# facebookresearch/SlowFast

Hardware: NVIDIA H100
Metric: clips/sec (fwd+bwd) SlowFast-8x8-R50 (higher is better)
Workload: dtype bf16x3-split operands, f32 accumulate/storage

## Files before the change

### slowfast_b200/csrc/conv_igemm.cu

```cuda
#include <algorithm>
#include <cstdint>
#include <cstdio>

#include "../../include/slowfast_b200.h"
#include "ptx.cuh"
#include "runtime.h"

namespace sfb {

constexpr int BLOCK_M = 128;
constexpr int MAX_STAGES = 8;
constexpr int CONV_THREADS = 384;
constexpr int PRODUCER_REGS = 40;
constexpr int CONSUMER_REGS = 232;
constexpr int BAR_ORDER = 1;
constexpr int BAR_EPI = 3;
constexpr int BN_MAX = 128;
constexpr int BLOCK_K = 64;
constexpr int KSTEPS = BLOCK_K / 16;
constexpr long long kNoRow = INT64_MIN;
constexpr uint32_t EPI_SCRATCH = BLOCK_M * 8 + 4 * 8 * 32 * 4;
static_assert(4 * BN_MAX * 2 * 4 <= 4 * 8 * 32 * 4, "BatchNorm partials fit the staging blocks");

struct ConvParams {
  CUtensorMap tmA[2];
  CUtensorMap tmB[2];
  int M, oq, op, oz, nb;
  int sw, sh, sd;
  int lw, lh, ld;
  int kw, kh, kd;
  int dw, dh, dd;
  int CK, cpt, n_chunks, cps, k_blocks;
  int Ntot, BN, n_tiles, m_tiles;
  int ksplit;
  int stages;
  int a_tiled;
  uint32_t stage_bytes, chunk_bytes, b_bytes, a_total_bytes, a_plane_bytes;
  uint32_t a_layout, a_sbo, a_lbo;
  uint32_t a_kstep[KSTEPS];
  uint32_t off_epi, off_bars;
  float* out;
  long long os_n, os_z, os_p, os_q;
  int accumulate;
  float* stats;
};

__device__ __forceinline__ int k_block_begin(const ConvParams& p, int kpart) {
  return kpart * p.k_blocks / p.ksplit;
}

int conv_direct_try(const sfb_conv_desc* d, cudaStream_t stream, int* rc_out);

template <int BN, int MODE>
__device__ __forceinline__ void store_fragment(const float (&d)[2][BN / 2], float* stage, const long long* roff,
                                               float* out, int ncols) {
  const int warp = (threadIdx.x >> 5) & 3, lane = threadIdx.x & 31;
  const int g = lane >> 2, cq = 2 * (lane & 3);
  const int rr = lane >> 3, c4 = 4 * (lane & 7);
#pragma unroll
  for (int rb = 0; rb < 2; ++rb) {
#pragma unroll
    for (int h = 0; h < 2; ++h) {
#pragma unroll
      for (int cg = 0; cg < (BN + 31) / 32; ++cg) {
#pragma unroll
        for (int jj = 0; jj < 4; ++jj) {
          const int jn = 4 * cg + jj;
          if (jn < BN / 8)
            *reinterpret_cast<float2*>(stage + g * 32 + ((8 * jj + cq) ^ (8 * (g & 3)))) =
                make_float2(d[rb][4 * jn + 2 * h], d[rb][4 * jn + 2 * h + 1]);
        }
        __syncwarp();
        float4 v[2];
#pragma unroll
        for (int k = 0; k < 2; ++k) v[k] = *reinterpret_cast<const float4*>(stage + (rr + 4 * k) * 32 + (c4 ^ (8 * rr)));
        __syncwarp();
        const int col = 32 * cg + c4;
        if (col >= ncols) continue;
        float4* dst[2];
        bool ok[2];
#pragma unroll
        for (int k = 0; k < 2; ++k) {
          const long long o = roff[64 * rb + 16 * warp + 8 * h + rr + 4 * k];
          ok[k] = o != kNoRow;
          dst[k] = reinterpret_cast<float4*>(out + (ok[k] ? o + col : 0));
        }
        if (MODE == 1) {
          float4 o[2];
#pragma unroll
          for (int k = 0; k < 2; ++k)
            if (ok[k]) o[k] = *dst[k];
#pragma unroll
          for (int k = 0; k < 2; ++k)
            if (ok[k]) *dst[k] = make_float4(v[k].x + o[k].x, v[k].y + o[k].y, v[k].z + o[k].z, v[k].w + o[k].w);
        } else {
#pragma unroll
          for (int k = 0; k < 2; ++k) {
            if (!ok[k]) continue;
            if (MODE == 2)
              asm volatile("red.global.add.v4.f32 [%0], {%1, %2, %3, %4};" ::"l"(dst[k]), "f"(v[k].x), "f"(v[k].y),
                           "f"(v[k].z), "f"(v[k].w) : "memory");
            else
              *dst[k] = v[k];
          }
        }
      }
    }
  }
}

template <int NSPLIT, int BN>
__global__ void __launch_bounds__(CONV_THREADS, 1) conv_igemm_kernel(const __grid_constant__ ConvParams p) {
  static_assert(BN % 16 == 0 && BN <= BN_MAX, "tile width: a multiple of 16 up to BN_MAX");
  extern __shared__ uint8_t smem_raw[];
  uint8_t* smem = reinterpret_cast<uint8_t*>((reinterpret_cast<uintptr_t>(smem_raw) + 1023) & ~uintptr_t(1023));

  uint64_t* full = reinterpret_cast<uint64_t*>(smem + p.off_bars);
  uint64_t* empty = full + MAX_STAGES;

  if (threadIdx.x == 0) {
    for (int s = 0; s < p.stages; ++s) {
      mbar_init(&full[s], 1);
      mbar_init(&empty[s], 128);
    }
    fence_mbar_init();
    fence_proxy_async_smem();
  }
  __syncthreads();

  const int total_units = p.m_tiles * p.n_tiles * p.ksplit;

  if (threadIdx.x < 128) {
    setmaxnreg_dec<PRODUCER_REGS>();
    if (threadIdx.x >= 32) return;
    if (threadIdx.x == 0) {
      tma_prefetch_desc(&p.tmA[0]);
      tma_prefetch_desc(&p.tmB[0]);
      if (NSPLIT == 3) {
        tma_prefetch_desc(&p.tmA[1]);
        tma_prefetch_desc(&p.tmB[1]);
      }
    }
    int stage = 0;
    uint32_t phase = 0;
    for (int unit = blockIdx.x; unit < total_units; unit += gridDim.x) {
      const int tile = unit / p.ksplit, kpart = unit - tile * p.ksplit;
      const int mt = tile / p.n_tiles, nt = tile - mt * p.n_tiles;
      const int kb0 = k_block_begin(p, kpart), kb1 = k_block_begin(p, kpart + 1);
      int t = mt * BLOCK_M;
      const int q0 = t % p.oq;
      t /= p.oq;
      const int p0 = t % p.op;
      t /= p.op;
      const int z0 = t % p.oz;
      const int n0 = t / p.oz;
      const int cw = p.lw + q0 * p.sw, ch = p.lh + p0 * p.sh, cd = p.ld + z0 * p.sd;
      for (int kb = kb0; kb < kb1; ++kb) {
        mbar_wait(&empty[stage], phase ^ 1);
        if (elect_one()) {
          const int chunk0 = kb * p.cps;
          const uint32_t bytes = (uint32_t(p.cps) * p.chunk_bytes + p.b_bytes) * (NSPLIT == 3 ? 2u : 1u);
          mbar_expect_tx(&full[stage], bytes);
          uint8_t* st = smem + size_t(stage) * p.stage_bytes;
          for (int j = 0; j < p.cps; ++j) {
            const int idx = chunk0 + j;
            int nn = p.nb, c0 = 0;
            uint16_t ow = 0, oh = 0, od = 0;
            if (idx < p.n_chunks) {
              const int tap = idx / p.cpt;
              c0 = (idx - tap * p.cpt) * p.CK;
              const int tw = tap % p.kw;
              const int t2 = tap / p.kw;
              const int th = t2 % p.kh;
              const int td = t2 / p.kh;
              ow = uint16_t(tw * p.dw);
              oh = uint16_t(th * p.dh);
              od = uint16_t(td * p.dd);
              nn = n0;
            }
            if (p.a_tiled) {
              const int row0 = idx < p.n_chunks ? mt * BLOCK_M : p.m_tiles * BLOCK_M;
              tma_load_2d(st + j * p.chunk_bytes, &p.tmA[0], &full[stage], c0, row0);
              if (NSPLIT == 3) tma_load_2d(st + p.a_plane_bytes + j * p.chunk_bytes, &p.tmA[1], &full[stage], c0, row0);
              continue;
            }
            tma_load_im2col_5d(st + j * p.chunk_bytes, &p.tmA[0], &full[stage], c0, cw, ch, cd, nn, ow, oh, od);
            if (NSPLIT == 3)
              tma_load_im2col_5d(st + p.a_plane_bytes + j * p.chunk_bytes, &p.tmA[1], &full[stage], c0, cw, ch, cd,
                                 nn, ow, oh, od);
          }
          tma_load_2d(st + p.a_total_bytes, &p.tmB[0], &full[stage], kb * 64, nt * BN);
          if (NSPLIT == 3)
            tma_load_2d(st + p.a_total_bytes + p.b_bytes, &p.tmB[1], &full[stage], kb * 64, nt * BN);
        }
        __syncwarp();
        if (++stage == p.stages) {
          stage = 0;
          phase ^= 1;
        }
      }
    }
    return;
  }

  setmaxnreg_inc<CONSUMER_REGS>();
  const int c = (threadIdx.x >> 7) - 1;
  const int t = threadIdx.x & 127, warp = t >> 5, lane = t & 31;
  const uint32_t a_rb = (8u * p.a_sbo) >> 4;
  float d[2][BN / 2];
  int stage = 0;
  uint32_t phase = 0;
  for (int j = 0, unit = blockIdx.x; unit < total_units; ++j, unit += gridDim.x) {
    const int tile = unit / p.ksplit, kpart = unit - tile * p.ksplit;
    const int kb0 = k_block_begin(p, kpart), kb1 = k_block_begin(p, kpart + 1);
    if ((j & 1) != c) {
      for (int kb = kb0; kb < kb1; ++kb) {
        if (++stage == p.stages) {
          stage = 0;
          phase ^= 1;
        }
      }
      continue;
    }
    if (j > 0) named_bar_sync(BAR_ORDER + c, 256);
#pragma unroll
    for (int i = 0; i < BN / 2; ++i) d[0][i] = d[1][i] = 0.f;
    int held = -1;
    for (int kb = kb0; kb < kb1; ++kb) {
      mbar_wait(&full[stage], phase);
      wgmma_fence();
      const uint32_t a_base = smem_u32(smem + size_t(stage) * p.stage_bytes);
      const uint32_t b_base = a_base + p.a_total_bytes;
      const uint64_t a_hi0 = make_smem_desc(a_base, p.a_lbo, p.a_sbo, p.a_layout);
      const uint64_t b_hi0 = make_smem_desc(b_base, 16, 1024, 2);
#pragma unroll
      for (int ks = 0; ks < KSTEPS; ++ks) {
        const uint64_t a_hi = a_hi0 + p.a_kstep[ks];
        const uint64_t b_hi = b_hi0 + uint64_t(ks * 2);
        if (NSPLIT == 3) {
          const uint64_t a_lo = a_hi + (p.a_plane_bytes >> 4);
          const uint64_t b_lo = b_hi + (p.b_bytes >> 4);
          wgmma_m64n<BN>(d[0], a_lo, b_hi);
          wgmma_m64n<BN>(d[1], a_lo + a_rb, b_hi);
          wgmma_m64n<BN>(d[0], a_hi, b_lo);
          wgmma_m64n<BN>(d[1], a_hi + a_rb, b_lo);
        }
        wgmma_m64n<BN>(d[0], a_hi, b_hi);
        wgmma_m64n<BN>(d[1], a_hi + a_rb, b_hi);
      }
      wgmma_commit();
      wgmma_wait<1>();
      if (held >= 0) mbar_arrive(&empty[held]);
      held = stage;
      if (++stage == p.stages) {
        stage = 0;
        phase ^= 1;
      }
    }
    if (unit + int(gridDim.x) < total_units) named_bar_arrive(BAR_ORDER + (c ^ 1), 256);

    const int mt = tile / p.n_tiles, nt = tile - mt * p.n_tiles;
    const int ncol0 = nt * BN;
    uint8_t* epi = smem + p.off_epi + size_t(c) * EPI_SCRATCH;
    long long* roff_s = reinterpret_cast<long long*>(epi);
    {
      int r = mt * BLOCK_M + t;
      long long off = kNoRow;
      if (r < p.M) {
        const int oq_ = r % p.oq;
        r /= p.oq;
        const int op_ = r % p.op;
        r /= p.op;
        const int oz_ = r % p.oz;
        const int on_ = r / p.oz;
        off = on_ * p.os_n + oz_ * p.os_z + op_ * p.os_p + oq_ * p.os_q;
      }
      roff_s[t] = off;
    }
    named_bar_sync(BAR_EPI + c, 128);
    const int cq = 2 * (lane & 3);
    const int ncols = min(BN, ((p.Ntot + 3) & ~3) - ncol0);
    float* stage_w = reinterpret_cast<float*>(epi + BLOCK_M * 8) + warp * 256;
    wgmma_wait<0>();
    mbar_arrive(&empty[held]);
    if (p.accumulate == 2) store_fragment<BN, 2>(d, stage_w, roff_s, p.out + ncol0, ncols);
    else if (p.accumulate == 1) store_fragment<BN, 1>(d, stage_w, roff_s, p.out + ncol0, ncols);
    else store_fragment<BN, 0>(d, stage_w, roff_s, p.out + ncol0, ncols);
    if (p.stats != nullptr) {
      float* red = reinterpret_cast<float*>(epi + BLOCK_M * 8);
      named_bar_sync(BAR_EPI + c, 128);
#pragma unroll
      for (int jn = 0; jn < BN / 8; ++jn) {
        float s[2], q[2];
#pragma unroll
        for (int e = 0; e < 2; ++e) {
          const float a0 = d[0][4 * jn + e], a1 = d[0][4 * jn + 2 + e], a2 = d[1][4 * jn + e], a3 = d[1][4 * jn + 2 + e];
          s[e] = (a0 + a1) + (a2 + a3);
          q[e] = fmaf(a0, a0, fmaf(a1, a1, fmaf(a2, a2, a3 * a3)));
#pragma unroll
          for (int o = 4; o <= 16; o <<= 1) {
            s[e] += __shfl_xor_sync(0xffffffffu, s[e], o);
            q[e] += __shfl_xor_sync(0xffffffffu, q[e], o);
          }
        }
        if (lane < 4)
          *reinterpret_cast<float4*>(red + (size_t(warp) * BN + 8 * jn + cq) * 2) = make_float4(s[0], q[0], s[1], q[1]);
      }
      named_bar_sync(BAR_EPI + c, 128);
      const int col = ncol0 + t;
      if (t < BN && col < p.Ntot) {
        float s = 0.f, s2 = 0.f;
#pragma unroll
        for (int w = 0; w < 4; ++w) {
          s += red[(size_t(w) * BN + t) * 2 + 0];
          s2 += red[(size_t(w) * BN + t) * 2 + 1];
        }
        p.stats[size_t(col) * p.m_tiles + mt] = s;
        p.stats[(size_t(p.Ntot) + col) * p.m_tiles + mt] = s2;
      }
      named_bar_sync(BAR_EPI + c, 128);
    }
  }
}

static int pick_ck(int c) {
  if (c % 64 == 0) return 64;
  if (c % 32 == 0) return 32;
  if (c % 16 == 0) return 16;
  return 8;
}

struct ConvGrid {
  int64_t M;
  int CK, cps, n_chunks, k_blocks, BN, m_tiles, n_tiles;
};
static ConvGrid conv_grid(const sfb_conv_desc* d) {
  ConvGrid g;
  g.M = int64_t(d->n) * d->out_t * d->out_h * d->out_w;
  g.CK = pick_ck(d->c);
  g.cps = BLOCK_K / g.CK;
  g.n_chunks = d->kt * d->kh * d->kw * (d->c / g.CK);
  g.k_blocks = (g.n_chunks + g.cps - 1) / g.cps;
  g.BN = std::min((d->cout + 15) / 16 * 16, BN_MAX);
  g.m_tiles = int((g.M + BLOCK_M - 1) / BLOCK_M);
  g.n_tiles = (d->cout + g.BN - 1) / g.BN;
  return g;
}

static bool rows_regular(const sfb_conv_desc* d) {
  return d->os_h == int64_t(d->out_w) * d->os_w && d->os_t == int64_t(d->out_h) * d->os_h &&
         d->os_n == int64_t(d->out_t) * d->os_t;
}

static int conv_ksplit(const sfb_conv_desc* d, const ConvGrid& g, int P, bool with_stats) {
  const int tiles = g.m_tiles * g.n_tiles;
  if (P <= 0 || d->c <= 8 || 2 * tiles < P) return 1;
  if ((d->accumulate == 0 || with_stats) && !rows_regular(d)) return 1;
  if (with_stats && (d->accumulate != 0 || d->cout % 8 != 0 || d->os_w % 4 != 0)) return 1;
  auto cost = [&](int s) { return double((int64_t(tiles) * s + P - 1) / P) / s * (1.0 + 0.02 * (s - 1)); };
  int best = 1;
  for (int s = 2; s <= 8 && 4 * s <= g.k_blocks; ++s)
    if (cost(s) < cost(best)) best = s;
  return cost(best) < 0.9 * cost(1) ? best : 1;
}

}

using namespace sfb;

extern "C" int64_t sfb_conv_m_tiles(const sfb_conv_desc* d) {
  const ConvGrid g = conv_grid(d);
  int sms = 0;
  if (device_limits(&sms, nullptr) == 0 && conv_ksplit(d, g, sms, true) > 1)
    return sfb_bn_split_stats_tiles(g.M, g.M, 1, d->cout);
  return g.m_tiles;
}

extern "C" int32_t sfb_conv_ksplit(const sfb_conv_desc* d) {
  int sms = 0;
  if (device_limits(&sms, nullptr)) return 1;
  return conv_ksplit(d, conv_grid(d), sms, d->stats != nullptr);
}

extern "C" int sfb_conv_igemm(const sfb_conv_desc* d, void* stream_) {
  cudaStream_t stream = reinterpret_cast<cudaStream_t>(stream_);
  int num_sms = 0, smem_optin = 0;
  if (device_limits(&num_sms, &smem_optin)) return -1;
  if (d->nsplit != 1 && d->nsplit != 3) {
    set_error("sfb_conv_igemm: nsplit must be 1 or 3 (got %d)", d->nsplit);
    return -10;
  }
  if (d->c % 8 != 0 || d->c_pitch % 8 != 0 || d->c <= 0) {
    set_error("sfb_conv_igemm: channel count %d / pitch %lld must be positive multiples of 8", d->c,
              (long long)d->c_pitch);
    return -10;
  }
  if (!d->a_hi || !d->b_hi || !d->out || (d->nsplit == 3 && (!d->a_lo || !d->b_lo))) {
    set_error("sfb_conv_igemm: null operand pointer");
    return -10;
  }
  const int64_t M64 = int64_t(d->n) * d->out_t * d->out_h * d->out_w;
  if (M64 <= 0 || M64 > 0x7fffffffLL || d->cout <= 0) {
    set_error("sfb_conv_igemm: bad output extent M=%lld cout=%d", (long long)M64, d->cout);
    return -10;
  }

  {
    int rc_direct = 0;
    if (conv_direct_try(d, stream, &rc_direct)) return rc_direct;
  }
  ConvParams p;
  memset(&p, 0, sizeof(p));
  p.M = int(M64);
  p.oq = d->out_w;
  p.op = d->out_h;
  p.oz = d->out_t;
  p.nb = d->n;
  p.sw = d->str_w;
  p.sh = d->str_h;
  p.sd = d->str_t;
  p.lw = d->low_w;
  p.lh = d->low_h;
  p.ld = d->low_t;
  p.kw = d->kw;
  p.kh = d->kh;
  p.kd = d->kt;
  p.dw = d->dil_w;
  p.dh = d->dil_h;
  p.dd = d->dil_t;
  const ConvGrid g = conv_grid(d);
  const int taps = d->kt * d->kh * d->kw;
  p.CK = g.CK;
  p.cpt = d->c / p.CK;
  p.n_chunks = g.n_chunks;
  p.cps = g.cps;
  p.k_blocks = g.k_blocks;
  p.Ntot = d->cout;
  p.BN = g.BN;
  p.n_tiles = g.n_tiles;
  p.m_tiles = g.m_tiles;
  p.ksplit = conv_ksplit(d, g, num_sms, d->stats != nullptr);
  p.chunk_bytes = BLOCK_M * p.CK * 2;
  p.b_bytes = p.BN * 128;
  p.a_plane_bytes = (uint32_t(p.cps) * p.chunk_bytes + 1023u) / 1024u * 1024u;
  p.a_total_bytes = p.a_plane_bytes * (d->nsplit == 3 ? 2 : 1);
  p.stage_bytes = p.a_total_bytes + p.b_bytes * (d->nsplit == 3 ? 2 : 1);
  p.stage_bytes = (p.stage_bytes + 1023) / 1024 * 1024;
  switch (p.CK) {
    case 64: p.a_layout = 2; p.a_sbo = 1024; p.a_lbo = 16; break;
    case 32: p.a_layout = 4; p.a_sbo = 512; p.a_lbo = 16; break;
    case 16: p.a_layout = 6; p.a_sbo = 256; p.a_lbo = 16; break;
    default: p.a_layout = 0; p.a_sbo = 128; p.a_lbo = p.chunk_bytes; break;
  }
  for (int ks = 0; ks < KSTEPS; ++ks) {
    const int k0 = ks * 16;
    const uint32_t off = p.CK >= 16 ? uint32_t(k0 / p.CK) * p.chunk_bytes + uint32_t(k0 % p.CK) * 2u
                                    : uint32_t(ks * 2) * p.chunk_bytes;
    p.a_kstep[ks] = off >> 4;
  }
  const uint32_t epi_bytes = 2u * EPI_SCRATCH;
  const uint32_t budget = uint32_t(smem_optin) - 1024 - epi_bytes - 256;
  p.stages = std::min<int>(MAX_STAGES, budget / p.stage_bytes);
  p.stages = std::min(p.stages, std::max(2, p.k_blocks * 4));
  const int ctas_per_sm = 1;
  if (p.stages < 2) {
    set_error("sfb_conv_igemm: not enough shared memory for 2 pipeline stages (stage=%u B)", p.stage_bytes);
    return -11;
  }
  p.off_epi = p.stages * p.stage_bytes;
  p.off_bars = p.off_epi + epi_bytes;
  const uint32_t smem_bytes = p.off_bars + 256 + 1024;
  p.out = d->out;
  p.os_n = d->os_n;
  p.os_z = d->os_t;
  p.os_p = d->os_h;
  p.os_q = d->os_w;
  p.accumulate = p.ksplit > 1 ? 2 : d->accumulate;
  p.stats = p.ksplit > 1 ? nullptr : d->stats;

  const int lower[3] = {d->low_w, d->low_h, d->low_t};
  const int strd[3] = {d->str_w, d->str_h, d->str_t};
  const int upper[3] = {d->low_w + (d->out_w - 1) * d->str_w + 1 - d->w, d->low_h + (d->out_h - 1) * d->str_h + 1 - d->h,
                        d->low_t + (d->out_t - 1) * d->str_t + 1 - d->d};
  const SwizzleBytes aswz = p.CK == 64 ? SWZ_128 : p.CK == 32 ? SWZ_64 : p.CK == 16 ? SWZ_32 : SWZ_NONE;
  p.a_tiled = (taps == 1 && d->str_w == 1 && d->str_h == 1 && d->str_t == 1 && d->low_w == 0 && d->low_h == 0 &&
               d->low_t == 0 && d->out_w == d->w && d->out_h == d->h && d->out_t == d->d)
                  ? 1 : 0;
  int rc;
  if (p.a_tiled)
    rc = make_tmap_2d_bf16(&p.tmA[0], d->a_hi, uint64_t(p.M), uint64_t(d->c), uint64_t(d->c_pitch), BLOCK_M, p.CK, aswz);
  else
    rc = make_tmap_im2col_bf16(&p.tmA[0], d->a_hi, d->n, d->d, d->h, d->w, d->c, d->c_pitch, lower, upper, strd, p.CK,
                               BLOCK_M, aswz);
  if (rc) return rc;
  const uint64_t ktot = uint64_t(taps) * d->c;
  rc = make_tmap_2d_bf16(&p.tmB[0], d->b_hi, d->cout, ktot, ktot, p.BN, 64, SWZ_128);
  if (rc) return rc;
  if (d->nsplit == 3) {
    if (p.a_tiled)
      rc = make_tmap_2d_bf16(&p.tmA[1], d->a_lo, uint64_t(p.M), uint64_t(d->c), uint64_t(d->c_pitch), BLOCK_M, p.CK, aswz);
    else
      rc = make_tmap_im2col_bf16(&p.tmA[1], d->a_lo, d->n, d->d, d->h, d->w, d->c, d->c_pitch, lower, upper, strd,
                                 p.CK, BLOCK_M, aswz);
    if (rc) return rc;
    rc = make_tmap_2d_bf16(&p.tmB[1], d->b_lo, d->cout, ktot, ktot, p.BN, 64, SWZ_128);
    if (rc) return rc;
  }

  if (p.ksplit > 1 && d->accumulate == 0) {
    const size_t width = size_t((d->cout + 3) & ~3) * sizeof(float);
    if (cudaMemset2DAsync(d->out, size_t(d->os_w) * sizeof(float), 0, width, size_t(p.M), stream) != cudaSuccess) {
      set_error("sfb_conv_igemm: zero fill of the split-K output failed: %s", cudaGetErrorString(cudaGetLastError()));
      return -20;
    }
  }
  const int units = p.m_tiles * p.n_tiles * p.ksplit;
  const int grid = std::min(units, num_sms * ctas_per_sm);
  {
    typedef void (*KernelFn)(const ConvParams);
#define SFB_CONV_FNS(S) {conv_igemm_kernel<S, 16>, conv_igemm_kernel<S, 32>, conv_igemm_kernel<S, 48>, \
                         conv_igemm_kernel<S, 64>, conv_igemm_kernel<S, 80>, conv_igemm_kernel<S, 96>, \
                         conv_igemm_kernel<S, 112>, conv_igemm_kernel<S, 128>}
    static const KernelFn fns[2][BN_MAX / 16] = {SFB_CONV_FNS(1), SFB_CONV_FNS(3)};
#undef SFB_CONV_FNS
    static bool attr[2][BN_MAX / 16] = {};
    const int a = d->nsplit == 3 ? 1 : 0, b = p.BN / 16 - 1;
    if (!attr[a][b]) {
      cudaFuncSetAttribute(fns[a][b], cudaFuncAttributeMaxDynamicSharedMemorySize, smem_optin);
      attr[a][b] = true;
    }
    fns[a][b]<<<grid, CONV_THREADS, smem_bytes, stream>>>(p);
  }
  if (int rc = launch_status("sfb_conv_igemm", "grid=%d smem=%u stages=%d BN=%d CK=%d ksplit=%d", grid, smem_bytes,
                             p.stages, p.BN, p.CK, p.ksplit))
    return rc;
  if (p.ksplit > 1 && d->stats != nullptr)
    return sfb_bn_split_stats(d->out, d->os_w, p.M, d->cout, 1, p.M, d->stats, stream);
  return 0;
}
```

Baseline: 193.7.

## Add halo-tiled narrow-channel convolution kernel for small Cin/Cout layers

Adds a specialized convolution path for layers with 16 or 32 input channels and at most 16 output channels. It loads a spatio-temporal halo patch once into shared memory with double-buffered cp.async and reuses it across all kernel taps with mma.sync, rather than going through the general TMA implicit-GEMM with 128-wide tiles. This is meant to cut wasted tile work and redundant input traffic on the thin fast-pathway layers. The cost is a second code path to maintain, and the per-CTA stats layout may differ from the main kernel's.

```diff
diff --git a/slowfast_b200/csrc/conv_igemm.cu b/slowfast_b200/csrc/conv_igemm.cu
--- a/slowfast_b200/csrc/conv_igemm.cu
+++ b/slowfast_b200/csrc/conv_igemm.cu
@@ -50,6 +50,7 @@
 }
 
 int conv_direct_try(const sfb_conv_desc* d, cudaStream_t stream, int* rc_out);
+int conv_narrow_try(const sfb_conv_desc* d, cudaStream_t stream, int* rc_out);
 
 template <int BN, int MODE>
 __device__ __forceinline__ void store_fragment(const float (&d)[2][BN / 2], float* stage, const long long* roff,
@@ -408,6 +409,7 @@
   {
     int rc_direct = 0;
     if (conv_direct_try(d, stream, &rc_direct)) return rc_direct;
+    if (conv_narrow_try(d, stream, &rc_direct)) return rc_direct;
   }
   ConvParams p;
   memset(&p, 0, sizeof(p));
diff --git a/slowfast_b200/csrc/conv_narrow.cu b/slowfast_b200/csrc/conv_narrow.cu
--- /dev/null
+++ b/slowfast_b200/csrc/conv_narrow.cu
@@ -0,0 +1,361 @@
+#include <algorithm>
+#include <cstdint>
+#include <cuda_bf16.h>
+
+#include "../../include/slowfast_b200.h"
+#include "ptx.cuh"
+#include "runtime.h"
+
+namespace sfb {
+
+constexpr int NARROW_THREADS = 256;
+constexpr int NARROW_ROWS = 128;
+constexpr uint32_t NARROW_HALO_MAX = 64 * 1024;
+constexpr int NARROW_BN = 16;
+
+struct NarrowPlan {
+  int pt, ph, pw;
+  int gt, gh, gw;
+  int ht, hh, hw;
+  int64_t tiles;
+};
+
+struct NarrowParams {
+  const __nv_bfloat16* a[2];
+  const __nv_bfloat16* b[2];
+  long long c_pitch;
+  int nb, id, ih, iw;
+  int cpp_log2;
+  int cout, kch;
+  int kt, kh, kw, st, sh, sw, lt, lh, lw, ot, oh, ow;
+  int pt, ph, pw, gt, gh, gw, ht, hh, hw;
+  int tiles;
+  int m_tiles;
+  uint32_t halo_plane, b_plane, b_pitch;
+  uint32_t off_halo, off_red;
+  float* out;
+  long long os_n, os_t, os_h, os_w;
+  int accumulate, ncols;
+  float* stats;
+};
+
+__device__ __forceinline__ void nw_cp_async16(uint32_t dst, const void* src, uint32_t bytes) {
+  asm volatile("cp.async.cg.shared.global [%0], [%1], 16, %2;" ::"r"(dst), "l"(src), "r"(bytes) : "memory");
+}
+__device__ __forceinline__ void nw_cp_commit() { asm volatile("cp.async.commit_group;" ::: "memory"); }
+template <int N>
+__device__ __forceinline__ void nw_cp_wait() {
+  asm volatile("cp.async.wait_group %0;" ::"n"(N) : "memory");
+}
+__device__ __forceinline__ void ldsm_x4(uint32_t addr, uint32_t (&r)[4]) {
+  asm volatile("ldmatrix.sync.aligned.m8n8.x4.shared.b16 {%0, %1, %2, %3}, [%4];"
+               : "=r"(r[0]), "=r"(r[1]), "=r"(r[2]), "=r"(r[3])
+               : "r"(addr)
+               : "memory");
+}
+__device__ __forceinline__ void mma_bf16_16816(float (&d)[4], const uint32_t (&a)[4], uint32_t b0, uint32_t b1) {
+  asm volatile(
+      "mma.sync.aligned.m16n8k16.row.col.f32.bf16.bf16.f32 {%0, %1, %2, %3}, {%4, %5, %6, %7}, {%8, %9}, "
+      "{%0, %1, %2, %3};"
+      : "+f"(d[0]), "+f"(d[1]), "+f"(d[2]), "+f"(d[3])
+      : "r"(a[0]), "r"(a[1]), "r"(a[2]), "r"(a[3]), "r"(b0), "r"(b1));
+}
+__device__ __forceinline__ uint32_t halo_swizzle(uint32_t L) { return L ^ ((L >> 3) & 7u); }
+
+struct PatchPos {
+  int n, t0, h0, w0;
+};
+__device__ __forceinline__ PatchPos patch_pos(const NarrowParams& p, int tile) {
+  PatchPos q;
+  const int xw = tile % p.gw;
+  tile /= p.gw;
+  const int xh = tile % p.gh;
+  tile /= p.gh;
+  const int xt = tile % p.gt;
+  q.n = tile / p.gt;
+  q.t0 = xt * p.pt;
+  q.h0 = xh * p.ph;
+  q.w0 = xw * p.pw;
+  return q;
+}
+
+template <int NSPLIT>
+__device__ __forceinline__ void load_halo(const NarrowParams& p, uint32_t dst, int tile) {
+  const PatchPos q = patch_pos(p, tile);
+  const int z0 = p.lt + q.t0 * p.st, y0 = p.lh + q.h0 * p.sh, x0 = p.lw + q.w0 * p.sw;
+  const int cpp_mask = (1 << p.cpp_log2) - 1;
+  const int chunks = (p.ht * p.hh * p.hw) << p.cpp_log2;
+  for (int L = threadIdx.x; L < chunks; L += NARROW_THREADS) {
+    const int px = L >> p.cpp_log2, j = L & cpp_mask;
+    const int x = px % p.hw, yz = px / p.hw;
+    const int y = yz % p.hh, z = yz / p.hh;
+    const int gz = z0 + z, gy = y0 + y, gx = x0 + x;
+    const bool in = unsigned(gz) < unsigned(p.id) && unsigned(gy) < unsigned(p.ih) && unsigned(gx) < unsigned(p.iw);
+    const long long off = in ? (((int64_t(q.n) * p.id + gz) * p.ih + gy) * p.iw + gx) * p.c_pitch + j * 8 : 0;
+    const uint32_t s = dst + (halo_swizzle(uint32_t(L)) << 4);
+    nw_cp_async16(s, p.a[0] + off, in ? 16u : 0u);
+    if (NSPLIT == 3) nw_cp_async16(s + p.halo_plane, p.a[1] + off, in ? 16u : 0u);
+  }
+}
+
+template <int NSPLIT, int BN>
+__global__ void __launch_bounds__(NARROW_THREADS, 2) conv_narrow_kernel(const __grid_constant__ NarrowParams p) {
+  extern __shared__ __align__(128) uint8_t nsm[];
+  const int tid = threadIdx.x, warp = tid >> 5, lane = tid & 31;
+  const uint32_t sbase = smem_u32(nsm);
+  const uint32_t halo0 = sbase + p.off_halo;
+  const uint32_t halo_buf = p.halo_plane * (NSPLIT == 3 ? 2u : 1u);
+  float* red = reinterpret_cast<float*>(nsm + p.off_red);
+
+  for (int L = tid; L < BN * p.kch; L += NARROW_THREADS) {
+    const int r = L / p.kch, c = L - r * p.kch;
+    const bool in = r < p.cout;
+    const size_t off = in ? (size_t(r) * p.kch + c) * 8 : 0;
+    const uint32_t s = sbase + ((uint32_t(r) * p.b_pitch + c) << 4);
+    nw_cp_async16(s, p.b[0] + off, in ? 16u : 0u);
+    if (NSPLIT == 3) nw_cp_async16(s + p.b_plane, p.b[1] + off, in ? 16u : 0u);
+  }
+  int tile = blockIdx.x;
+  if (tile < p.tiles) load_halo<NSPLIT>(p, halo0, tile);
+  nw_cp_commit();
+
+  const int P = p.pt * p.ph * p.pw;
+  int hp = 0;
+  {
+    const int r = 16 * warp + (lane & 15);
+    if (r < P) {
+      const int rw = r % p.pw, rh = (r / p.pw) % p.ph, rt = r / (p.pw * p.ph);
+      hp = ((rt * p.st) * p.hh + rh * p.sh) * p.hw + rw * p.sw;
+    }
+  }
+  const int khalf = lane >> 4;
+  const uint32_t brow = (lane & 7) + ((lane >> 4) << 3);
+  const uint32_t bhalf = (lane >> 3) & 1;
+  const int ksteps = (1 << p.cpp_log2) >> 1;
+  const uint32_t bsm = sbase + ((brow * p.b_pitch + bhalf) << 4);
+
+  float cta_s = 0.f, cta_s2 = 0.f;
+  for (int it = 0; tile < p.tiles; ++it, tile += gridDim.x) {
+    __syncthreads();
+    const int next = tile + gridDim.x;
+    if (next < p.tiles) load_halo<NSPLIT>(p, halo0 + ((it + 1) & 1) * halo_buf, next);
+    nw_cp_commit();
+    nw_cp_wait<1>();
+    __syncthreads();
+
+    const uint32_t halo = halo0 + (it & 1) * halo_buf;
+    float acc[BN / 8][4];
+#pragma unroll
+    for (int j = 0; j < BN / 8; ++j) acc[j][0] = acc[j][1] = acc[j][2] = acc[j][3] = 0.f;
+    int kc = 0;
+    for (int dt = 0; dt < p.kt; ++dt)
+      for (int dh = 0; dh < p.kh; ++dh)
+        for (int dw = 0; dw < p.kw; ++dw) {
+          const uint32_t row = uint32_t(hp + (dt * p.hh + dh) * p.hw + dw) << p.cpp_log2;
+          for (int ks = 0; ks < ksteps; ++ks, kc += 2) {
+            const uint32_t aaddr = halo + (halo_swizzle(row + 2 * ks + khalf) << 4);
+            uint32_t ah[4], al[4];
+            ldsm_x4(aaddr, ah);
+            if (NSPLIT == 3) ldsm_x4(aaddr + p.halo_plane, al);
+#pragma unroll
+            for (int np = 0; np < BN / 16; ++np) {
+              const uint32_t baddr = bsm + ((uint32_t(16 * np) * p.b_pitch + kc) << 4);
+              uint32_t bh[4], bl[4];
+              ldsm_x4(baddr, bh);
+              if (NSPLIT == 3) {
+                ldsm_x4(baddr + p.b_plane, bl);
+                mma_bf16_16816(acc[2 * np], al, bh[0], bh[1]);
+                mma_bf16_16816(acc[2 * np + 1], al, bh[2], bh[3]);
+                mma_bf16_16816(acc[2 * np], ah, bl[0], bl[1]);
+                mma_bf16_16816(acc[2 * np + 1], ah, bl[2], bl[3]);
+              }
+              mma_bf16_16816(acc[2 * np], ah, bh[0], bh[1]);
+              mma_bf16_16816(acc[2 * np + 1], ah, bh[2], bh[3]);
+            }
+          }
+        }
+
+    const PatchPos q = patch_pos(p, tile);
+    long long roff[2];
+    bool ok[2];
+#pragma unroll
+    for (int h = 0; h < 2; ++h) {
+      const int r = 16 * warp + (lane >> 2) + 8 * h;
+      const int rw = r % p.pw, rh = (r / p.pw) % p.ph, rt = r / (p.pw * p.ph);
+      const int t = q.t0 + rt, y = q.h0 + rh, x = q.w0 + rw;
+      ok[h] = r < P && t < p.ot && y < p.oh && x < p.ow;
+      roff[h] = ok[h] ? q.n * p.os_n + t * p.os_t + y * p.os_h + x * p.os_w : 0;
+    }
+    const int cq = 2 * (lane & 3);
+#pragma unroll
+    for (int j = 0; j < BN / 8; ++j) {
+      const int col = 8 * j + cq;
+      if (col >= p.ncols) continue;
+#pragma unroll
+      for (int h = 0; h < 2; ++h) {
+        if (!ok[h]) continue;
+        float2* dst = reinterpret_cast<float2*>(p.out + roff[h] + col);
+        float2 v = make_float2(acc[j][2 * h], acc[j][2 * h + 1]);
+        if (p.accumulate == 2) {
+          asm volatile("red.global.add.v2.f32 [%0], {%1, %2};" ::"l"(dst), "f"(v.x), "f"(v.y) : "memory");
+        } else {
+          if (p.accumulate == 1) {
+            const float2 o = *dst;
+            v.x += o.x;
+            v.y += o.y;
+          }
+          *dst = v;
+        }
+      }
+    }
+    if (p.stats != nullptr) {
+#pragma unroll
+      for (int j = 0; j < BN / 8; ++j) {
+        float s[2], s2[2];
+#pragma unroll
+        for (int e = 0; e < 2; ++e) {
+          const float a0 = ok[0] ? acc[j][e] : 0.f, a1 = ok[1] ? acc[j][2 + e] : 0.f;
+          s[e] = a0 + a1;
+          s2[e] = fmaf(a0, a0, a1 * a1);
+#pragma unroll
+          for (int o = 4; o <= 16; o <<= 1) {
+            s[e] += __shfl_xor_sync(0xffffffffu, s[e], o);
+            s2[e] += __shfl_xor_sync(0xffffffffu, s2[e], o);
+          }
+        }
+        if (lane < 4)
+          *reinterpret_cast<float4*>(red + (size_t(warp) * BN + 8 * j + cq) * 2) = make_float4(s[0], s2[0], s[1], s2[1]);
+      }
+      __syncthreads();
+      if (tid < BN) {
+#pragma unroll
+        for (int w = 0; w < NARROW_THREADS / 32; ++w) {
+          cta_s += red[(size_t(w) * BN + tid) * 2 + 0];
+          cta_s2 += red[(size_t(w) * BN + tid) * 2 + 1];
+        }
+      }
+    }
+  }
+  nw_cp_wait<0>();
+  if (p.stats != nullptr && tid < p.cout) {
+    for (int col = blockIdx.x; col < p.m_tiles; col += gridDim.x) {
+      const bool mine = col == int(blockIdx.x);
+      p.stats[size_t(tid) * p.m_tiles + col] = mine ? cta_s : 0.f;
+      p.stats[(size_t(p.cout) + tid) * p.m_tiles + col] = mine ? cta_s2 : 0.f;
+    }
+  }
+}
+
+static int64_t cdiv(int64_t a, int64_t b) { return (a + b - 1) / b; }
+
+static bool narrow_plan(const sfb_conv_desc* d, NarrowPlan* pl) {
+  const int taps = d->kt * d->kh * d->kw;
+  if (d->nsplit != 1 && d->nsplit != 3) return false;
+  if (d->dil_t != 1 || d->dil_h != 1 || d->dil_w != 1) return false;
+  if (d->c != 16 && d->c != 32) return false;
+  if (d->cout <= 0 || d->cout > NARROW_BN || d->c > 32 || (d->c == 32 && taps == 1) || taps > 9) return false;
+  if (d->c_pitch % 8 != 0 || d->out_w > NARROW_ROWS) return false;
+  const uintptr_t a_align = uintptr_t(d->a_hi) | uintptr_t(d->a_lo) | uintptr_t(d->b_hi) | uintptr_t(d->b_lo);
+  if (a_align % 16 != 0) return false;
+  if ((uintptr_t(d->out) | uintptr_t(d->os_n | d->os_t | d->os_h | d->os_w) * 4) % 8 != 0) return false;
+  const int planes = d->nsplit == 3 ? 2 : 1;
+  const int bn = NARROW_BN;
+  bool found = false;
+  int64_t best = 0;
+  int tc[8], nt = 0, hc[8], nh = 0;
+  for (int v = 1; v < d->out_t && v <= 64; v <<= 1) tc[nt++] = v;
+  tc[nt++] = d->out_t;
+  for (int v = 1; v < d->out_h && v <= 64; v <<= 1) hc[nh++] = v;
+  hc[nh++] = d->out_h;
+  const int wc[4] = {d->out_w, 32, 16, 8};
+  for (int i = 0; i < 4; ++i) {
+    const int pw = wc[i];
+    if (pw > d->out_w || (i > 0 && pw == d->out_w)) continue;
+    for (int a = 0; a < nh; ++a) {
+      const int ph = hc[a];
+      for (int b = 0; b < nt; ++b) {
+        const int pt = tc[b];
+        if (int64_t(pt) * ph * pw > NARROW_ROWS) break;
+        const int ht = (pt - 1) * d->str_t + d->kt, hh = (ph - 1) * d->str_h + d->kh, hw = (pw - 1) * d->str_w + d->kw;
+        const int64_t bytes = int64_t(ht) * hh * hw * d->c * 2 * planes;
+        if (bytes > NARROW_HALO_MAX) continue;
+        const int64_t tiles = int64_t(d->n) * cdiv(d->out_t, pt) * cdiv(d->out_h, ph) * cdiv(d->out_w, pw);
+        const int64_t cost = tiles * (bytes + 512 * bn + 8192);
+        if (!found || cost < best) {
+          found = true;
+          best = cost;
+          *pl = NarrowPlan{pt, ph, pw, int(cdiv(d->out_t, pt)), int(cdiv(d->out_h, ph)), int(cdiv(d->out_w, pw)),
+                           ht, hh, hw, tiles};
+        }
+      }
+    }
+  }
+  return found && pl->tiles <= 0x7fffffffLL;
+}
+
+int conv_narrow_try(const sfb_conv_desc* d, cudaStream_t stream, int* rc_out) {
+  NarrowPlan pl;
+  if (!narrow_plan(d, &pl)) return 0;
+  int num_sms = 0, smem_optin = 0;
+  if (device_limits(&num_sms, &smem_optin)) {
+    *rc_out = -1;
+    return 1;
+  }
+  const int planes = d->nsplit == 3 ? 2 : 1;
+  const int taps = d->kt * d->kh * d->kw;
+  NarrowParams p;
+  p.a[0] = static_cast<const __nv_bfloat16*>(d->a_hi);
+  p.a[1] = static_cast<const __nv_bfloat16*>(d->a_lo);
+  p.b[0] = static_cast<const __nv_bfloat16*>(d->b_hi);
+  p.b[1] = static_cast<const __nv_bfloat16*>(d->b_lo);
+  p.c_pitch = d->c_pitch;
+  p.nb = d->n; p.id = d->d; p.ih = d->h; p.iw = d->w;
+  p.cpp_log2 = 0;
+  while ((8 << p.cpp_log2) < d->c) ++p.cpp_log2;
+  p.cout = d->cout;
+  p.kch = taps * d->c / 8;
+  p.kt = d->kt; p.kh = d->kh; p.kw = d->kw;
+  p.st = d->str_t; p.sh = d->str_h; p.sw = d->str_w;
+  p.lt = d->low_t; p.lh = d->low_h; p.lw = d->low_w;
+  p.ot = d->out_t; p.oh = d->out_h; p.ow = d->out_w;
+  p.pt = pl.pt; p.ph = pl.ph; p.pw = pl.pw;
+  p.gt = pl.gt; p.gh = pl.gh; p.gw = pl.gw;
+  p.ht = pl.ht; p.hh = pl.hh; p.hw = pl.hw;
+  p.tiles = int(pl.tiles);
+  p.m_tiles = int((int64_t(d->n) * d->out_t * d->out_h * d->out_w + NARROW_ROWS - 1) / NARROW_ROWS);
+  p.halo_plane = uint32_t((int64_t(pl.ht) * pl.hh * pl.hw * (d->c / 8) + 7) / 8 * 8 * 16);
+  p.b_pitch = uint32_t(p.kch | 1);
+  p.b_plane = uint32_t(NARROW_BN) * p.b_pitch * 16u;
+  p.off_halo = (p.b_plane * planes + 127u) / 128u * 128u;
+  p.off_red = p.off_halo + 2u * p.halo_plane * planes;
+  const uint32_t smem = p.off_red + uint32_t(NARROW_THREADS / 32) * NARROW_BN * 2 * 4;
+  p.out = d->out;
+  p.os_n = d->os_n; p.os_t = d->os_t; p.os_h = d->os_h; p.os_w = d->os_w;
+  p.accumulate = d->accumulate;
+  p.ncols = (d->cout + 3) & ~3;
+  p.stats = d->stats;
+  if (smem > uint32_t(smem_optin)) {
+    set_error("sfb_conv_igemm (narrow body): %u B of shared memory exceed the device's %d", smem, smem_optin);
+    *rc_out = -11;
+    return 1;
+  }
+
+  typedef void (*KernelFn)(const NarrowParams);
+  static const KernelFn fns[2] = {conv_narrow_kernel<1, NARROW_BN>, conv_narrow_kernel<3, NARROW_BN>};
+  static bool attr[2] = {};
+  const int a = d->nsplit == 3 ? 1 : 0;
+  if (!attr[a]) {
+    cudaFuncSetAttribute(fns[a], cudaFuncAttributeMaxDynamicSharedMemorySize, smem_optin);
+    attr[a] = true;
+  }
+  int per_sm = 1;
+  if (cudaOccupancyMaxActiveBlocksPerMultiprocessor(&per_sm, fns[a], NARROW_THREADS, smem) != cudaSuccess || per_sm < 1)
+    per_sm = 1;
+  const int grid = int(std::min<int64_t>(std::min<int64_t>(pl.tiles, p.m_tiles), int64_t(num_sms) * per_sm));
+  fns[a]<<<grid, NARROW_THREADS, smem, stream>>>(p);
+  *rc_out = launch_status("sfb_conv_igemm (narrow halo-tile body)", "grid=%d smem=%u patch=%dx%dx%d", grid, smem,
+                          pl.pt, pl.ph, pl.pw);
+  return 1;
+}
+
+}
```

After: 195.2 (median of 6 runs). Within noise of the previous version (+0.8%).
